# totokunda/apex-studio

Measured on AMD Instinct MI355X. Metric: denoise_steps_per_sec, higher is better.
Workload: dtype bf16; 1 GPU; flux-dev-1024x1024 denoise step (19 double + 38 single MM-DiT blocks, S_img 4096 + S_txt 512, B=1, no CFG) + FlowMatch-Euler step; clips_in_flight=1, parallelism=clip-per-gpu x1

## Files before the change

### apex-studio_amd/csrc/common.h

```cpp
#pragma once
#include <hip/hip_runtime.h>
#include <stdint.h>
#include <stddef.h>

#include "../../include/apexmi.h"

typedef __attribute__((ext_vector_type(8))) __bf16 bf16x8;
typedef __attribute__((ext_vector_type(4))) __bf16 bf16x4;
typedef __attribute__((ext_vector_type(2))) __bf16 bf16x2;
typedef __attribute__((ext_vector_type(16))) float f32x16;
typedef __attribute__((ext_vector_type(4))) float f32x4;
typedef __attribute__((ext_vector_type(2))) float f32x2;
typedef __attribute__((ext_vector_type(4))) uint32_t u32x4;
typedef __attribute__((ext_vector_type(2))) uint32_t u32x2;

typedef uint16_t bf16_t;

#define APEXMI_DEVICE __device__ __forceinline__

APEXMI_DEVICE float bf16_lo(uint32_t u) { return __uint_as_float(u << 16); }
APEXMI_DEVICE float bf16_hi(uint32_t u) { return __uint_as_float(u & 0xffff0000u); }
APEXMI_DEVICE float bf16_to_f32(bf16_t b) { return __uint_as_float((uint32_t)b << 16); }

APEXMI_DEVICE uint32_t pack_bf16(float a, float b) {
// ... 123 lines not shown
}
APEXMI_DEVICE float sum_xor32(float x) {
    float a, b;
    swap32(x, a, b);
    return a + b;
}

APEXMI_DEVICE float wave_sum(float x) {
#pragma unroll
    for (int o = 32; o > 0; o >>= 1) x += __shfl_xor(x, o, 64);
    return x;
}
APEXMI_DEVICE float wave_max(float x) {
#pragma unroll
    for (int o = 32; o > 0; o >>= 1) x = fmaxf(x, __shfl_xor(x, o, 64));
    return x;
}

APEXMI_DEVICE float fast_exp2(float x) { return __builtin_amdgcn_exp2f(x); }
APEXMI_DEVICE float x_sigmoid_log2(float x, float z_log2) {
    return x * __builtin_amdgcn_rcpf(1.0f + __builtin_amdgcn_exp2f(-z_log2));
}
APEXMI_DEVICE float silu_f(float x) { return x_sigmoid_log2(x, 1.4426950408889634f * x); }
APEXMI_DEVICE float gelu_tanh_f(float x) {
    const float a = 2.0f * 0.7978845608028654f * 1.4426950408889634f, b = a * 0.044715f;
    return x_sigmoid_log2(x, x * fmaf(b, x * x, a));
}

APEXMI_DEVICE void glds16(const void* gsrc, void* lds) {
    __builtin_amdgcn_global_load_lds((const __attribute__((address_space(1))) void*)gsrc,
                                     (__attribute__((address_space(3))) void*)lds, 16, 0, 0);
}

APEXMI_DEVICE int xcd_remap(int bid, int total) {
    const int q = total >> 3, r = total & 7;
    const int xcd = bid & 7, idx = bid >> 3;
    const int base = (xcd < r) ? xcd * (q + 1) : r * (q + 1) + (xcd - r) * q;
    return base + idx;
}

static inline bool apexmi_attr_needed(const uint64_t& mask) {
    int dev = 0;
    (void)hipGetDevice(&dev);
    return dev >= 64 || !(__atomic_load_n(&mask, __ATOMIC_ACQUIRE) & (1ull << dev));
}
static inline void apexmi_attr_done(uint64_t& mask) {
    int dev = 0;
    (void)hipGetDevice(&dev);
    if (dev < 64) (void)__atomic_fetch_or(&mask, 1ull << dev, __ATOMIC_RELEASE);
}
#define APEXMI_SET_ATTR_ONCE(mask, ...)      \
    do {                                     \
        if (apexmi_attr_needed(mask)) {      \
            __VA_ARGS__;                     \
            apexmi_attr_done(mask);          \
        }                                    \
    } while (0)
void apexmi_set_error(const char* fmt, ...);
int apexmi_check_launch(const char* what);
__attribute__((visibility("hidden"))) int apexmi_attn_merge_f32(int n, const float* parts, const float* lses, void* out,
                                                                 float* lse_out, int B, int H, int Sq, int D,
                                                                 const int64_t* o_strides, const int64_t* lse_strides, int dtype,
                                                                 hipStream_t stream);
unsigned long long* apexmi_clk_ptr();

struct ApexmiProfScope {
    int cls;
// ... 14 lines not shown
```

### apex-studio_amd/csrc/gemm.hip

```cpp
#include "common.h"

#include <cstring>
#include <type_traits>

namespace {

#ifndef APEXMI_GEMM_TRACE
#define APEXMI_GEMM_TRACE 0
#endif
#define PP_BAR()                               \
    do {                                       \
        __builtin_amdgcn_sched_barrier(0);     \
        __builtin_amdgcn_s_barrier();          \
        __builtin_amdgcn_sched_barrier(0);     \
    } while (0)
#define PP_SYNC()                                                                   \
    do {                                                                            \
        asm volatile("s_waitcnt lgkmcnt(0)" ::: "memory");                          \
        PP_BAR();                                                                   \
    } while (0)
#define VMCNT(n) asm volatile("s_waitcnt vmcnt(" #n ")" ::: "memory")
constexpr int BK = 64;
constexpr int GROUP_M = 6;
constexpr int EPI_GATE_RES_F32 = 7;
constexpr int MAX_GROUPS = 4;

struct GemmProblem {
    const bf16_t* A;
    const bf16_t* W;
    const bf16_t* bias;
    bf16_t* C;
    const float* gate;
    const bf16_t* R;
    int64_t lda, ldw, ldc, ldr;
    int M, N, nm, nn, tile0, gelu;
    int qkv, row0;
    const bf16_t* nq;
    const bf16_t* nk;
};
struct QkvShared {
    bf16_t* qo;
    bf16_t* ko;
    bf16_t* vt;
    const float* rope;
    int S_out, Skp, inner;
    float eps;
    const float* rope_pairs;
};
struct GemmGroup {
    GemmProblem p[MAX_GROUPS];
    int count, K, total, group_m;
    int batch;
    int64_t bsA, bsW, bsC_bytes;
    QkvShared qs;
    unsigned long long* clk;
#if APEXMI_GEMM_TRACE
    unsigned long long* trace;
#endif
    int wpacked;
};

template <int BM_, int BN_, int WM_, int WN_, int SCHED_>
struct Cfg {
    static constexpr int BM = BM_, BN = BN_, WM = WM_, WN = WN_;
    static constexpr int SCHED = SCHED_;
    static constexpr bool PP = SCHED_ == 1;
    static constexpr int NW = WM * WN, NT = NW * 64;
    static constexpr int TM = BM / WM / 32, TN = BN / WN / 32;
    static constexpr int A_BYTES = BM * BK * 2, W_BYTES = BN * BK * 2;
    static constexpr int STAGE = A_BYTES + W_BYTES;
    static constexpr int LDS = SCHED_ == 8 ? 5 * 32768 : 2 * STAGE;
    static constexpr int A_LD = BM * 8 / NT, W_LD = BN * 8 / NT;
    static constexpr int OCC = (LDS <= 80 * 1024 && NT == 256) ? 2 : (NT == 512 ? 2 : 1);
};
using CFG_128 = Cfg<128, 128, 2, 2, 0>;
using CFG_256 = Cfg<256, 256, 2, 4, 0>;
using CFG_128E = Cfg<128, 128, 2, 4, 0>;
using CFG_256P = Cfg<256, 256, 2, 4, 1>;
using CFG_256W = Cfg<256, 256, 2, 2, 4>;
using CFG_256P16 = Cfg<256, 256, 2, 4, 5>;
using CFG_256R = Cfg<256, 256, 2, 4, 7>;
using CFG_256R5 = Cfg<256, 256, 2, 4, 8>;

APEXMI_DEVICE float act_f(float x, int mode) {
    if (mode == 1) return gelu_tanh_f(x);
    if (mode == 2) return 0.5f * x * (1.0f + erff(x * 0.70710678118654752f));
    if (mode == 4) return x_sigmoid_log2(x, (1.702f * 1.4426950408889634f) * x);
    return silu_f(x);
}
template <int ACT>
APEXMI_DEVICE float act_c(float x) {
    if constexpr (ACT == 0) return x;
// ... 473 lines not shown
            if (!(APEXMI_QK_ABL & 16) && (MT > 8 || (mt & 1))) __builtin_amdgcn_sched_barrier(0);
        }
    }
}

#if APEXMI_GEMM_TRACE
#define APEXMI_TRACE_END()                                                                                   \
    do {                                                                                                     \
        if (G.trace != nullptr) {                                                                            \
            __builtin_amdgcn_sched_barrier(0);                                                               \
            const unsigned long long t_st = __builtin_amdgcn_s_memrealtime();                                \
            asm volatile("s_waitcnt vmcnt(0)" ::: "memory");                                                 \
            const unsigned long long t_ack = __builtin_amdgcn_s_memrealtime();                               \
            if (tid == 0) {                                                                                  \
                unsigned long long* o = G.trace + (size_t)blockIdx.x * 8;                                    \
                o[0] = __builtin_amdgcn_s_getreg((31 << 11) | (0 << 6) | 4);               \
                o[1] = __builtin_amdgcn_s_getreg((31 << 11) | (0 << 6) | 20);             \
                o[2] = tr_in;                                                                                \
                o[3] = tr_l0;                                                                                \
                o[4] = tr_l1;                                                                                \
                o[5] = t_st;                                                                                 \
                o[6] = t_ack;                                                                                \
                o[7] = (unsigned long long)s;                                                                \
            }                                                                                                \
        }                                                                                                    \
    } while (0)
#else
#define APEXMI_TRACE_END() do { } while (0)
#endif

struct TileCoord {
    int pm, pn;
};
__device__ __forceinline__ TileCoord tile_coord(int s, int nm, int nn, int group_m) {
    const int width = group_m * nn;
    const int first_m = (s / width) * group_m;
    const int gsz = min(nm - first_m, group_m);
    return TileCoord{first_m + (s % width) % gsz, (s % width) / gsz};
}

__device__ __forceinline__ const char* uniform_ptr(const char* p) {
    const uint64_t u = (uint64_t)p;
    const uint32_t hi = __builtin_amdgcn_readfirstlane((uint32_t)(u >> 32)), lo = __builtin_amdgcn_readfirstlane((uint32_t)u);
    return (const char*)(((uint64_t)hi << 32) | lo);
}
#pragma clang diagnostic push
#pragma clang diagnostic ignored "-Winline-asm"
__device__ __forceinline__ void glds16_s(const char* sbase, uint32_t voff, uint32_t la) {
    asm volatile("s_mov_b32 m0, %2\n\ts_nop 0\n\tglobal_load_lds_dwordx4 %0, %1"
                 :: "v"(voff), "s"(sbase), "s"(la) : "memory", "m0");
}
#pragma clang diagnostic pop

struct KRange {
    int kt0, kt1;
};
template <typename CFG, int EPI>
__device__ __forceinline__ void gemm_tile(const GemmGroup& G, char* smem, int s, const KRange& kr) {
    constexpr int BM = CFG::BM, BN = CFG::BN, TM = CFG::TM, TN = CFG::TN;

#if APEXMI_GEMM_TRACE
    unsigned long long tr_in = 0, tr_l0 = 0, tr_l1 = 0;
    if (G.trace != nullptr) tr_in = __builtin_amdgcn_s_memrealtime();
#endif
    int tid_ = threadIdx.x;
    asm volatile("" : "+v"(tid_));
    const int tid = tid_;
    const int lane = tid & 63;
    const int wave = __builtin_amdgcn_readfirstlane(tid >> 6);
    const int wm = wave / CFG::WN, wn = wave % CFG::WN;
    const int l31 = lane & 31, hi = lane >> 5;
// ... 814 lines not shown
    }
    const int nbase = n0 + wn * 48;
    if constexpr (EPI == APEXMI_EPI_BIAS_GATE_RES) {
        u32x4 rr[9];
        u32x2 r1[9];
        const int nst = nbase + 16 * (g4 & 1) + 8 * (g4 >> 1);
#pragma unroll
        for (int mt = 0; mt < 9; ++mt) {
            const bf16_t* row = P.R + (int64_t)max(mrow[mt], 0) * P.ldr;
            rr[mt] = *(const u32x4*)(row + min(nst, N - 8));
            r1[mt] = *(const u32x2*)(row + min(nbase + 32 + 4 * g4, N - 4));
        }
        store_slab16<EPI, 9, 0>(acc[0], acc[1], P, N, mrow, nbase, g4, rr);
        store_single16<EPI, 9, 0>(acc[2], P, N, mrow, nbase + 32, g4, r1);
    } else {
        APEXMI_ACT_DISPATCH(P.gelu, store_slab16<EPI, 9, ACT>(acc[0], acc[1], P, N, mrow, nbase, g4);
                            store_single16<EPI, 9, ACT>(acc[2], P, N, mrow, nbase + 32, g4, nullptr));
    }
}

constexpr int YBM = 384, YBN = 256;
constexpr int Y_A_BYTES = YBM * BK * 2, Y_W_BYTES = YBN * BK * 2, Y_STAGE = Y_A_BYTES + Y_W_BYTES, Y_LDS = 2 * Y_STAGE;

template <int EPI, int DIST = 1, int QKV = 0>
__global__ __launch_bounds__(512, 2) void gemm_bf16_x384_kernel(const GemmGroup G) {
    extern __shared__ __attribute__((aligned(16))) char smem[];
    const int tid = threadIdx.x;
    const int lane = tid & 63;
    const int wave = __builtin_amdgcn_readfirstlane(tid >> 6);
    const int wm = wave >> 2, wn = wave & 3;

    int s = xcd_remap(blockIdx.x, G.total);
    int gi = 0;
#pragma unroll
    for (int i = 1; i < MAX_GROUPS; ++i)
        if (i < G.count && s >= G.p[i].tile0) gi = i;
    const GemmProblem P = G.p[gi];
    s -= P.tile0;
    const int N = P.N, M = P.M;
    const TileCoord tc = tile_coord(s, P.nm, P.nn, G.group_m);
    const int m0 = tc.pm * YBM, n0 = tc.pn * YBN;

    const int rows_a = min(M - m0, YBM), rows_w = min(N - n0, YBN);
    auto rsrc_a = __builtin_amdgcn_make_buffer_rsrc((void*)(P.A + (int64_t)m0 * P.lda), 0,
                                                    (int)(((int64_t)(rows_a - 1) * P.lda + G.K) * 2), 0x00020000);
    auto rsrc_w = __builtin_amdgcn_make_buffer_rsrc((void*)(P.W + (int64_t)n0 * P.ldw), 0,
                                                    (int)(((int64_t)(rows_w - 1) * P.ldw + G.K) * 2), 0x00020000);
    const int par = wave & 1, widx = wave >> 1;
    const int sw_src = ((lane & 7) ^ (4 * par + (lane >> 4))) * 16;
    const int voff_a = (lane >> 3) * (int)P.lda * 2 + sw_src;
    const int voff_w = (lane >> 3) * (int)P.ldw * 2 + sw_src;
    const int lda8 = (int)P.lda * 16, ldw8 = (int)P.ldw * 16;
    auto piece_of = [&](int j) -> int {
        if (j < 4) return 2 * (4 * j + widx) + par;
        const int e = 3 * widx + (j < 7 ? j - 4 : j - 7);
        return (e < 6 ? 0 : 24) + (j < 7 ? 0 : 12) + 2 * (e % 6) + par;
    };
    auto stage = [&](int buf, int kt, int j) {
        const int pc = piece_of(j);
        char* dst = smem + buf * Y_STAGE + (j < 4 ? Y_A_BYTES : 0) + pc * 1024;
        if (j < 4)
            __builtin_amdgcn_raw_ptr_buffer_load_lds(rsrc_w, (__attribute__((address_space(3))) void*)dst, 16, voff_w, pc * ldw8 + kt * (BK * 2), 0, 0);
        else
            __builtin_amdgcn_raw_ptr_buffer_load_lds(rsrc_a, (__attribute__((address_space(3))) void*)dst, 16, voff_a, pc * lda8 + kt * (BK * 2), 0, 0);
    };

    f32x4_t acc[4][12];
#pragma unroll
    for (int i = 0; i < 4; ++i)
#pragma unroll
        for (int j = 0; j < 12; ++j) acc[i][j] = f32x4_t{0.f, 0.f, 0.f, 0.f};

    const int nkt = G.K / BK;
// ... 135 lines not shown
        }
#pragma unroll
        for (int p = 0; p < 2; ++p) {
            const int nbase = n0 + wn * 64 + p * 32;
            const f32x4_t(&x)[MTC] = *(const f32x4_t(*)[MTC]) & acc[2 * p][h * MTC];
            const f32x4_t(&y)[MTC] = *(const f32x4_t(*)[MTC]) & acc[2 * p + 1][h * MTC];
            if constexpr (EPI == APEXMI_EPI_BIAS_GATE_RES) {
                u32x4 rr[MTC];
                const int nst = nbase + 16 * (g4 & 1) + 8 * (g4 >> 1);
#pragma unroll
                for (int mt = 0; mt < MTC; ++mt) rr[mt] = *(const u32x4*)(P.R + (int64_t)max(mrow[mt], 0) * P.ldr + min(nst, N - 8));
                store_slab16<EPI, MTC, 0>(x, y, P, N, mrow, nbase, g4, rr);
            } else {
                APEXMI_ACT_DISPATCH(P.gelu, store_slab16<EPI, MTC, ACT>(x, y, P, N, mrow, nbase, g4));
            }
        }
    }
    Y_TRACE_END(3);
}
#undef Y_TRACE_END

int g_group_m = GROUP_M;
#if APEXMI_GEMM_TRACE
uintptr_t g_gemm_trace = 0;
#endif
int g_large_cfg = 7;
int g_force_cfg = 0;
int g_wpacked = 0;
int g_tail_max = 96;
int g_x288 = 0;
int g_x384_group_m = 3;
int g_x384_dist = -1;
int g_x384_qkv = 1;
int g_x384 = 1;
int g_small_max = 112;
int g_tail_split = 2;

int number_tiles(GemmGroup& G, const int* Ms, int BM, int BN) {
    int t = 0;
    for (int i = 0; i < G.count; ++i) {
        G.p[i].M = Ms[i];
        G.p[i].nm = (Ms[i] + BM - 1) / BM;
        G.p[i].nn = (G.p[i].N + BN - 1) / BN;
        G.p[i].tile0 = t;
        t += G.p[i].nm * G.p[i].nn;
    }
    G.total = t;
    G.clk = apexmi_clk_ptr();
#if APEXMI_GEMM_TRACE
    G.trace = (unsigned long long*)g_gemm_trace;
#endif
    G.wpacked = 0;
    return t;
}

template <typename CFG, int EPI>
int launch_cfg(GemmGroup& G, const int* Ms, hipStream_t stream) {
    if constexpr (CFG::SCHED == 0 || CFG::SCHED == 5) {
        for (int i = 0; i < G.count; ++i)
            if (G.p[i].lda > (1 << 22) || G.p[i].ldw > (1 << 22)) {
                apexmi_set_error("gemm_bf16: leading dimensions above 2^22 elements are not supported (lda %lld, ldw %lld)",
                                 (long long)G.p[i].lda, (long long)G.p[i].ldw);
                return 1;
            }
    }
    static uint64_t attr_set = 0;
    APEXMI_SET_ATTR_ONCE(attr_set,
        (void)hipFuncSetAttribute((const void*)gemm_bf16_kernel<CFG, EPI>,
                                  hipFuncAttributeMaxDynamicSharedMemorySize, CFG::LDS));
    const int t = number_tiles(G, Ms, CFG::BM, CFG::BN);
    G.group_m = g_group_m;
    if (CFG::SCHED == 5) G.wpacked = g_wpacked;
    hipLaunchKernelGGL((gemm_bf16_kernel<CFG, EPI>), dim3(t, G.batch), dim3(CFG::NT), CFG::LDS, stream, G);
    return apexmi_check_launch("gemm_bf16");
}

template <int EPI>
int launch_x288(GemmGroup& G, const int* Ms, hipStream_t stream) {
    static uint64_t attr_set = 0;
    APEXMI_SET_ATTR_ONCE(attr_set,
        (void)hipFuncSetAttribute((const void*)gemm_bf16_x288_kernel<EPI>, hipFuncAttributeMaxDynamicSharedMemorySize, X_LDS));
    const int t = number_tiles(G, Ms, XBM, XBN);
    G.group_m = g_group_m;
    hipLaunchKernelGGL((gemm_bf16_x288_kernel<EPI>), dim3(t, 1), dim3(512), X_LDS, stream, G);
    return apexmi_check_launch("gemm_bf16 (288x192)");
}

template <int EPI>
int launch_x384(GemmGroup& G, const int* Ms, hipStream_t stream) {
    static uint64_t attr_set = 0;
    APEXMI_SET_ATTR_ONCE(attr_set,
        (void)hipFuncSetAttribute((const void*)gemm_bf16_x384_kernel<EPI, 0>, hipFuncAttributeMaxDynamicSharedMemorySize, Y_LDS);
        (void)hipFuncSetAttribute((const void*)gemm_bf16_x384_kernel<EPI, 1>, hipFuncAttributeMaxDynamicSharedMemorySize, Y_LDS);
        if constexpr (EPI == APEXMI_EPI_BIAS)
            (void)hipFuncSetAttribute((const void*)gemm_bf16_x384_kernel<EPI, 1, 1>, hipFuncAttributeMaxDynamicSharedMemorySize, Y_LDS));
    const int t = number_tiles(G, Ms, YBM, YBN);
    G.group_m = g_x384_group_m;
    bool any_qkv = false;
    for (int i = 0; i < G.count; ++i) any_qkv |= G.p[i].qkv != 0;
    if constexpr (EPI == APEXMI_EPI_BIAS) {
        if (any_qkv) {
            hipLaunchKernelGGL((gemm_bf16_x384_kernel<EPI, 1, 1>), dim3(t, 1), dim3(512), Y_LDS, stream, G);
            return apexmi_check_launch("gemm_bf16 (384x256, fused q/k/v)");
        }
    }
    const int dist = g_x384_dist >= 0 ? g_x384_dist : (t >= 2048 ? 0 : 1);
    if (dist == 0) hipLaunchKernelGGL((gemm_bf16_x384_kernel<EPI, 0>), dim3(t, 1), dim3(512), Y_LDS, stream, G);
    else hipLaunchKernelGGL((gemm_bf16_x384_kernel<EPI, 1>), dim3(t, 1), dim3(512), Y_LDS, stream, G);
    return apexmi_check_launch("gemm_bf16 (384x256)");
}

inline bool x288_pays(const GemmGroup& G, const int* Ms) {
    int64_t t256 = 0, t288 = 0;
    for (int i = 0; i < G.count; ++i) {
        if (G.p[i].qkv) return false;
        t256 += (int64_t)((Ms[i] + 255) / 256) * ((G.p[i].N + 255) / 256);
        t288 += (int64_t)((Ms[i] + XBM - 1) / XBM) * ((G.p[i].N + XBN - 1) / XBN);
    }
    const double c256 = (double)((t256 + 255) / 256) * 65536.0;
    const double c288 = (double)((t288 + 255) / 256) * (XBM * XBN) * 1.04;
    return c288 < 0.95 * c256;
}

inline bool use_x288(const GemmGroup& G, const int* Ms) {
    if (g_x288 == 0 || G.batch != 1 || G.K % BK != 0 || !(g_force_cfg == 0 || g_force_cfg == 7) || g_large_cfg != 7) return false;
    int64_t mtot = 0;
    int nmax = 0;
    for (int i = 0; i < G.count; ++i) {
        if (G.p[i].qkv) return false;
        mtot += Ms[i];
        nmax = G.p[i].N > nmax ? G.p[i].N : nmax;
    }
    if (g_x288 == 2) return true;
    return G.K >= 256 && mtot >= 1024 && nmax >= 1024 && x288_pays(G, Ms);
// ... 178 lines not shown
    double flops = 0, bytes = 0;
    const int kind = epi_kind(epilogue[0]);
    for (int i = 0; i < count; ++i) {
        APEXMI_REQUIRE(epi_kind(epilogue[i]) == kind,
                       "gemm_bf16_grouped: gate/residual (or float / bf16 output) problems cannot be mixed with the others");
        const float* g = gate ? gate[i] : nullptr;
        const void* r = R ? R[i] : nullptr;
        const int64_t lr = ldr ? ldr[i] : 0;
        if (int rc = check_problem(A[i], lda[i], W[i], ldw[i], C[i], ldc[i], M[i], N[i], K, epilogue[i], g, r, lr))
            return rc;
        G.p[i] = GemmProblem{(const bf16_t*)A[i], (const bf16_t*)W[i], (const bf16_t*)(bias ? bias[i] : nullptr),
                             (bf16_t*)C[i], g, (const bf16_t*)r, lda[i], ldw[i], ldc[i], lr, M[i], N[i], 0, 0, 0,
                             act_mode(epi_base(epilogue[i]))};
        flops += 2.0 * M[i] * N[i] * (double)K;
        bytes += 2.0 * ((double)M[i] * K + (double)N[i] * K + (double)M[i] * N[i]);
    }
    ApexmiProfScope prof(0, stream, flops, bytes);
    return launch_group(G, M, kind, stream);
}

extern "C" int apexmi_gemm_uses_x288(int M, int N, int K) {
    GemmGroup G;
    memset(&G, 0, sizeof(G));
    G.count = 1;
    G.K = K;
    G.batch = 1;
    G.p[0].N = N;
    return (M > 0 && N > 0 && K > 0 && use_x288(G, &M)) ? 1 : 0;
}

extern "C" int apexmi_gemm_qkv_fusable(int64_t m_total, int n_max, int K) {
    return (g_force_cfg == 0 || g_force_cfg == 7 || g_force_cfg == 9 || g_force_cfg == 10) &&
           (g_large_cfg == 7 || g_large_cfg == 9 || g_large_cfg == 10) && m_total >= 1024 && n_max >= 1024 && K >= 256 && K % BK == 0;
}

extern "C" int apexmi_gemm_bf16_grouped_qkv(int count, const void* const* A, const int64_t* lda, const void* const* W,
                                            const int64_t* ldw, const void* const* bias, void* const* C, const int64_t* ldc,
                                            const int* M, const int* N, int K, const int* epilogue, const int* is_qkv,
                                            const void* const* norm_q, const void* const* norm_k, const int* row0, int H,
                                            float eps, const float* rope, void* q_out, void* k_out, void* vt_out, int S_out,
                                            int Skp, apexmi_stream_t stream_) {
    return apexmi_gemm_bf16_grouped_qkv_pairs(count, A, lda, W, ldw, bias, C, ldc, M, N, K, epilogue, is_qkv, norm_q, norm_k, row0, H,
                                              eps, rope, nullptr, q_out, k_out, vt_out, S_out, Skp, stream_);
}

extern "C" int apexmi_gemm_bf16_grouped_qkv_pairs(int count, const void* const* A, const int64_t* lda, const void* const* W,
                                                  const int64_t* ldw, const void* const* bias, void* const* C, const int64_t* ldc,
                                                  const int* M, const int* N, int K, const int* epilogue, const int* is_qkv,
                                                  const void* const* norm_q, const void* const* norm_k, const int* row0, int H,
                                                  float eps, const float* rope, const float* rope_pairs, void* q_out, void* k_out,
                                                  void* vt_out, int S_out, int Skp, apexmi_stream_t stream_) {
    hipStream_t stream = (hipStream_t)stream_;
    APEXMI_REQUIRE(((uintptr_t)rope_pairs % 16) == 0, "gemm_bf16_grouped_qkv: rope_pairs must be 16-byte aligned");
    APEXMI_REQUIRE(count >= 1 && count <= MAX_GROUPS, "gemm_bf16_grouped_qkv: count=%d not in [1,%d]", count, MAX_GROUPS);
    APEXMI_REQUIRE(is_qkv && row0 && rope && q_out && k_out && vt_out && H > 0, "gemm_bf16_grouped_qkv: null argument");
    APEXMI_REQUIRE(H % 2 == 0 && S_out > 0 && Skp >= S_out && Skp % 8 == 0, "gemm_bf16_grouped_qkv: H=%d must be even, Skp=%d a multiple of 8 >= S_out=%d",
                   H, Skp, S_out);
    APEXMI_REQUIRE(((uintptr_t)rope % 16) == 0 && ((uintptr_t)q_out % 16) == 0 && ((uintptr_t)k_out % 16) == 0 && ((uintptr_t)vt_out % 16) == 0,
                   "gemm_bf16_grouped_qkv: rope / outputs must be 16-byte aligned");
    GemmGroup G;
    G.count = count;
    G.K = K;
    G.batch = 1;
    G.bsA = G.bsW = G.bsC_bytes = 0;
    G.qs = QkvShared{(bf16_t*)q_out, (bf16_t*)k_out, (bf16_t*)vt_out, rope, S_out, Skp, H * 128, eps, rope_pairs};
    double flops = 0, bytes = 0;
// ... 33 lines not shown
        return launch_x384<APEXMI_EPI_BIAS>(G, M, stream);
    if (g_large_cfg == 9 || g_force_cfg == 9) return launch_cfg<CFG_256R, APEXMI_EPI_BIAS>(G, M, stream);
    if (g_large_cfg == 10 || g_force_cfg == 10) return launch_cfg<CFG_256R5, APEXMI_EPI_BIAS>(G, M, stream);
    return launch_cfg<CFG_256P16, APEXMI_EPI_BIAS>(G, M, stream);
}

extern "C" int apexmi_split_bf16x3(const float* x, int64_t ldx, int64_t M, int K, void* out, int64_t ldo,
                                   apexmi_stream_t stream_) {
    hipStream_t stream = (hipStream_t)stream_;
    APEXMI_REQUIRE(x && out && M > 0 && K > 0, "split_bf16x3: bad arguments");
    APEXMI_REQUIRE(K % 8 == 0 && ldx % 4 == 0 && ldo % 8 == 0 && ldo >= 3 * (int64_t)K && ((uintptr_t)x % 16) == 0 &&
                       ((uintptr_t)out % 16) == 0,
                   "split_bf16x3: K=%d must be a multiple of 8 and rows 16-byte aligned", K);
    const int64_t n = M * (K / 8);
    ApexmiProfScope prof(5, stream, 0.0, 10.0 * (double)M * K);
    hipLaunchKernelGGL(split_bf16x3_kernel, dim3((unsigned)((n + 255) / 256)), dim3(256), 0, stream, x, ldx, M, K,
                       (bf16_t*)out, ldo);
    return apexmi_check_launch("split_bf16x3");
}

int apexmi_set_gemm_key(const char* key, int value) {
    if (!strcmp(key, "gemm.tail")) g_tail_split = value;
    else if (!strcmp(key, "gemm.tail_max")) g_tail_max = value;
    else if (!strcmp(key, "gemm.group_m")) g_group_m = value > 0 ? value : GROUP_M;
    else if (!strcmp(key, "gemm.large")) g_large_cfg = value;
    else if (!strcmp(key, "gemm.config")) g_force_cfg = value;
    else if (!strcmp(key, "gemm.wpacked")) g_wpacked = value;
    else if (!strcmp(key, "gemm.x288")) g_x288 = value;
    else if (!strcmp(key, "gemm.small_max")) g_small_max = value;
    else if (!strcmp(key, "gemm.x384")) g_x384 = value;
    else if (!strcmp(key, "gemm.x384_dist")) g_x384_dist = value;
    else if (!strcmp(key, "gemm.x384_group_m")) g_x384_group_m = value > 0 ? value : 3;
    else if (!strcmp(key, "gemm.x384_qkv")) g_x384_qkv = value;
#if APEXMI_GEMM_TRACE
    else if (!strcmp(key, "gemm.trace_lo")) g_gemm_trace = (g_gemm_trace & ~(uintptr_t)0xffffffffu) | (uint32_t)value;
    else if (!strcmp(key, "gemm.trace_hi")) g_gemm_trace = (g_gemm_trace & (uintptr_t)0xffffffffu) | ((uintptr_t)(uint32_t)value << 32);
#endif
    else return 1;
    return 0;
}
```

### apex-studio_amd/lib.py

```python
from __future__ import annotations

import ctypes as C
import os

_PKG_DIR = os.path.dirname(os.path.abspath(__file__))
LIB_PATH = os.environ.get("APEX_MI355_LIB") or os.path.join(_PKG_DIR, "libapex_mi355.so")

_lib = None

c_i64p = C.POINTER(C.c_int64)
c_f32p = C.c_void_p
vp = C.c_void_p

SIGNATURES = {
    "apexmi_version": (C.c_int, []),
    "apexmi_last_error": (C.c_char_p, []),
    "apexmi_attn_workspace_bytes": (C.c_size_t, [C.c_int] * 6),
    "apexmi_attn_fwd": (C.c_int, [vp, vp, vp, vp, C.c_int, C.c_int, C.c_int, C.c_int, C.c_int,
                                  c_i64p, c_i64p, c_i64p, c_i64p, C.c_float, C.c_int, vp,
                                  C.c_size_t, vp]),
    "apexmi_attn_fwd_prepared": (C.c_int, [vp, vp, vp, vp, C.c_int, C.c_int, C.c_int, C.c_int,
                                           C.c_int, c_i64p, C.c_float, vp]),
    "apexmi_attn_prepared_workspace_bytes": (C.c_size_t, [C.c_int] * 4),
    "apexmi_attn_fwd_prepared_ws": (C.c_int, [vp, vp, vp, vp, C.c_int, C.c_int, C.c_int, C.c_int,
# ... 15 lines not shown
                                                                                                C.c_float, C.c_int, vp, C.c_size_t, vp]),
    "apexmi_attn_merge": (C.c_int, [C.c_int, C.POINTER(vp), C.POINTER(vp), vp, vp] + [C.c_int] * 4 + [c_i64p, c_i64p, C.c_int, vp]),
    "apexmi_attn_varlen_workspace_bytes": (C.c_size_t, [C.c_int] * 4),
    "apexmi_attn_fwd_varlen": (C.c_int, [vp] * 7 + [C.c_int] * 8 + [c_i64p] * 5 + [C.c_int, C.c_float, C.c_int, vp, C.c_size_t, vp]),
    "apexmi_attn_window_map_bytes": (C.c_size_t, [C.c_int, C.c_int]),
    "apexmi_attn_window_map": (C.c_int, [vp, vp] + [C.c_int] * 5 + [vp, C.c_size_t, vp]),
    "apexmi_attn_fwd_window": (C.c_int, [vp, vp, vp, vp] + [C.c_int] * 6 + [c_i64p] * 4 + [vp, vp, C.c_int, C.c_int, C.c_int, vp,
                                                                                        C.c_float, C.c_int, vp, C.c_size_t, vp]),
    "apexmi_attn_fwd_prepared_window": (C.c_int, [vp, vp, vp, vp] + [C.c_int] * 5 + [c_i64p, vp, vp, C.c_int, C.c_int, C.c_int, vp,
                                                                                     C.c_float, vp]),
    "apexmi_attn_fwd_prepared_band": (C.c_int, [vp, vp, vp, vp] + [C.c_int] * 5 + [c_i64p, vp, C.c_int, C.c_float, vp]),
    "apexmi_attn_band_workspace_bytes": (C.c_size_t, [C.c_int] * 4),
    "apexmi_attn_fwd_band": (C.c_int, [vp, vp, vp, vp] + [C.c_int] * 5 + [c_i64p] * 4 + [vp, C.c_int, C.c_float, C.c_int, vp,
                                                                                      C.c_size_t, vp]),
    "apexmi_attn_fwd_prepared_dual": (C.c_int, [vp, vp, vp, C.c_int, C.c_int, vp, vp, C.c_int, C.c_int, vp, C.c_int, C.c_int,
                                                C.c_int, c_i64p, C.c_float, vp]),
    "apexmi_gemm_bf16": (C.c_int, [vp, C.c_int64, vp, C.c_int64, vp, vp, C.c_int64, C.c_int, C.c_int,
                                   C.c_int, C.c_int, vp, vp, C.c_int64, vp]),
    "apexmi_gemm_bf16_grouped": (C.c_int, [C.c_int, C.POINTER(vp), c_i64p, C.POINTER(vp), c_i64p,
                                           C.POINTER(vp), C.POINTER(vp), c_i64p, C.POINTER(C.c_int),
                                           C.POINTER(C.c_int), C.c_int, C.POINTER(C.c_int), C.POINTER(vp),
                                           C.POINTER(vp), c_i64p, vp]),
    "apexmi_gemm_bf16_grouped_qkv": (C.c_int, [C.c_int, C.POINTER(vp), c_i64p, C.POINTER(vp), c_i64p, C.POINTER(vp),
                                               C.POINTER(vp), c_i64p, C.POINTER(C.c_int), C.POINTER(C.c_int), C.c_int,
                                               C.POINTER(C.c_int), C.POINTER(C.c_int), C.POINTER(vp), C.POINTER(vp),
                                               C.POINTER(C.c_int), C.c_int, C.c_float, vp, vp, vp, vp, C.c_int, C.c_int, vp]),
    "apexmi_gemm_bf16_grouped_qkv_pairs": (C.c_int, [C.c_int, C.POINTER(vp), c_i64p, C.POINTER(vp), c_i64p, C.POINTER(vp),
                                                     C.POINTER(vp), c_i64p, C.POINTER(C.c_int), C.POINTER(C.c_int), C.c_int,
                                                     C.POINTER(C.c_int), C.POINTER(C.c_int), C.POINTER(vp), C.POINTER(vp),
                                                     C.POINTER(C.c_int), C.c_int, C.c_float, vp, vp, vp, vp, vp, C.c_int, C.c_int, vp]),
    "apexmi_rope_pairs": (C.c_int, [vp, C.c_int, C.c_int, vp, vp, vp]),
    "apexmi_gemm_qkv_fusable": (C.c_int, [C.c_int64, C.c_int, C.c_int]),
    "apexmi_gemm_uses_x288": (C.c_int, [C.c_int, C.c_int, C.c_int]),
    "apexmi_qk_rms_rope_rows": (C.c_int, [vp, vp, vp, C.c_int64, C.c_int, C.c_int, vp, vp, C.c_float, vp, C.c_int, vp, vp, vp,
                                          C.c_int, C.c_int, C.c_int, vp]),
    "apexmi_qk_rms_rope_rows_f32": (C.c_int, [vp, vp, vp, C.c_int64, C.c_int, C.c_int, vp, vp, C.c_float, vp, C.c_int, vp, vp, vp,
                                              C.c_int, C.c_int, C.c_int, vp]),
    "apexmi_gemm_bf16_batched": (C.c_int, [vp, C.c_int64, C.c_int64, vp, C.c_int64, C.c_int64, vp, C.c_int64, C.c_int64,
                                           C.c_int, C.c_int, C.c_int, C.c_int, C.c_int, vp]),
    "apexmi_attn_bias_workspace_bytes": (C.c_size_t, [C.c_int] * 4),
    "apexmi_attn_fwd_bias": (C.c_int, [vp, C.c_int64, vp, C.c_int64, vp, C.c_int64, vp, C.c_int64, C.c_int, C.c_int,
                                       C.c_int, C.c_int, C.c_int, C.c_float, vp, vp, vp, C.c_int, vp, C.c_size_t, vp]),
    "apexmi_rope_half": (C.c_int, [vp, C.c_int64, C.c_int64, C.c_int, C.c_int, C.c_int, vp, vp, vp]),
    "apexmi_rope_half_f32": (C.c_int, [vp, C.c_int64, C.c_int64, C.c_int, C.c_int, C.c_int, vp, vp, vp]),
    "apexmi_tune_set": (C.c_int, [C.c_char_p, C.c_int]),
    "apexmi_gemv": (C.c_int, [vp, C.c_int64, vp, vp, C.c_int64, vp, C.c_int64, C.c_int, C.c_int,
                              C.c_int, C.c_int, vp]),
    "apexmi_ln_modulate": (C.c_int, [vp, C.c_int64, vp, C.c_int64, C.c_int, C.c_int, vp, vp, vp, vp,
                                     C.c_float, C.c_int, vp]),
    "apexmi_ln_modulate2": (C.c_int, [vp, C.c_int64, vp, C.c_int64, C.c_int, C.c_int, vp, vp, vp, vp,
                                      C.c_float, C.c_int, C.c_int, vp, vp, vp]),
    "apexmi_qkv_prepare": (C.c_int, [vp, vp, vp, C.c_int64, C.c_int, C.c_int, C.c_int, C.c_int, vp, vp,
                                     vp, vp, C.c_float, vp, C.c_int, vp, vp, vp, C.c_int, C.c_int,
                                     C.c_int, vp]),
    "apexmi_v_transpose": (C.c_int, [vp, C.c_int64, C.c_int64, C.c_int, C.c_int, C.c_int, vp, C.c_int,
                                     C.c_int, vp]),
    "apexmi_conv3d_cl": (C.c_int, [vp, vp, vp, vp, vp, vp] + [C.c_int] * 9 + [vp]),
    "apexmi_conv3d_cl_replicate": (C.c_int, [vp, vp, vp, vp, vp, vp] + [C.c_int] * 9 + [vp]),
    "apexmi_conv3d_cl_clips": (C.c_int, [vp, vp, vp, vp, vp, vp] + [C.c_int] * 11 + [vp]),
    "apexmi_conv3d_cl_strided": (C.c_int, [vp, vp, vp, vp, vp, vp] + [C.c_int] * 15 + [vp]),
    "apexmi_conv3d_cl_frames": (C.c_int, [vp, vp, vp, vp, vp, vp] + [C.c_int] * 9 + [vp]),
    "apexmi_conv3d_cl_up2": (C.c_int, [vp, vp, vp, vp, vp, vp] + [C.c_int] * 10 + [vp]),
    "apexmi_conv3d_cl_norm_fusable": (C.c_int, [C.c_int] * 6),
    "apexmi_conv3d_cl_family": (C.c_int, [C.c_int] * 23 + [vp]),
    "apexmi_conv3d_cl_norm": (C.c_int, [vp, vp, vp, vp, vp, vp, vp, C.c_int, vp] + [C.c_int] * 11 + [vp]),
    "apexmi_add_bf16": (C.c_int, [vp, vp, vp, C.c_int64, vp]),
# ... 155 lines not shown
```

### include/apexmi.h

```cpp
#ifndef APEXMI_H
#define APEXMI_H

#include <stdint.h>
#include <stddef.h>

#ifdef __cplusplus
extern "C" {
#endif

typedef void* apexmi_stream_t;

#define APEXMI_BF16 0
#define APEXMI_F16 1
#define APEXMI_F32 2
#define APEXMI_MASK_BOOL 3

#define APEXMI_EPI_BIAS 0
#define APEXMI_EPI_BIAS_GELU 1
#define APEXMI_EPI_BIAS_GATE_RES 2
#define APEXMI_EPI_BIAS_GELU_ERF 4
#define APEXMI_EPI_BIAS_QUICK_GELU 6
#define APEXMI_EPI_BIAS_SILU 5
#define APEXMI_EPI_BIAS_F32 3

// ... 83 lines not shown
                           const int64_t o_strides[3], const void* q_coords, const void* k_coords, int r0, int r1, int r2,
                           const void* map, float softmax_scale, int dtype, void* workspace, size_t workspace_bytes,
                           apexmi_stream_t stream);
int apexmi_attn_fwd_prepared_window(const void* q, const void* k, const void* vt, void* out, int B, int H, int Sq, int Sk,
                                    int Skp, const int64_t o_strides[3], const void* q_coords, const void* k_coords, int r0,
                                    int r1, int r2, const void* map, float softmax_scale, apexmi_stream_t stream);

int apexmi_attn_fwd_prepared_band(const void* q, const void* k, const void* vt, void* out, int B, int H, int Sq, int Sk,
                                  int Skp, const int64_t o_strides[3], const void* bands, int Hb, float softmax_scale,
                                  apexmi_stream_t stream);
size_t apexmi_attn_band_workspace_bytes(int B, int H, int Sq, int Sk);
int apexmi_attn_fwd_band(const void* q, const void* k, const void* v, void* out, int B, int H, int Sq, int Sk, int D,
                         const int64_t q_strides[3], const int64_t k_strides[3], const int64_t v_strides[3],
                         const int64_t o_strides[3], const void* bands, int Hb, float softmax_scale, int dtype,
                         void* workspace, size_t workspace_bytes, apexmi_stream_t stream);

int apexmi_attn_fwd_prepared_dual(const void* q, const void* k_t, const void* vt_t, int Sk_t, int Skp_t, const void* k_i,
                                  const void* vt_i, int Sk_i, int Skp_i, void* out, int B, int H, int Sq,
                                  const int64_t o_strides[3], float softmax_scale, apexmi_stream_t stream);

int apexmi_gemm_bf16(const void* A, int64_t lda, const void* W, int64_t ldw, const void* bias,
                     void* C, int64_t ldc, int M, int N, int K, int epilogue,
                     const float* gate, const void* R, int64_t ldr, apexmi_stream_t stream);

int apexmi_gemm_uses_x288(int M, int N, int K);

int apexmi_gemm_bf16_grouped(int count, const void* const* A, const int64_t* lda,
                             const void* const* W, const int64_t* ldw, const void* const* bias,
                             void* const* C, const int64_t* ldc, const int* M, const int* N, int K,
                             const int* epilogue, const float* const* gate, const void* const* R,
                             const int64_t* ldr, apexmi_stream_t stream);

int apexmi_gemm_qkv_fusable(int64_t m_total, int n_max, int K);
int apexmi_gemm_bf16_grouped_qkv(int count, const void* const* A, const int64_t* lda, const void* const* W,
                                 const int64_t* ldw, const void* const* bias, void* const* C, const int64_t* ldc,
                                 const int* M, const int* N, int K, const int* epilogue, const int* is_qkv,
                                 const void* const* norm_q, const void* const* norm_k, const int* row0, int H, float eps,
                                 const float* rope, void* q_out, void* k_out, void* vt_out, int S_out, int Skp,
                                 apexmi_stream_t stream);
int apexmi_gemm_bf16_grouped_qkv_pairs(int count, const void* const* A, const int64_t* lda, const void* const* W,
                                       const int64_t* ldw, const void* const* bias, void* const* C, const int64_t* ldc,
                                       const int* M, const int* N, int K, const int* epilogue, const int* is_qkv,
                                       const void* const* norm_q, const void* const* norm_k, const int* row0, int H, float eps,
                                       const float* rope, const float* rope_pairs, void* q_out, void* k_out, void* vt_out,
                                       int S_out, int Skp, apexmi_stream_t stream);
int apexmi_rope_pairs(const float* rope, int S, int D, float* pairs, int* mismatch, apexmi_stream_t stream);

int apexmi_split_bf16x3(const float* x, int64_t ldx, int64_t M, int K, void* out, int64_t ldo, apexmi_stream_t stream);

int apexmi_gemm_bf16_batched(const void* A, int64_t lda, int64_t stride_a, const void* W, int64_t ldw, int64_t stride_w,
                             void* C, int64_t ldc, int64_t stride_c, int batch, int M, int N, int K, int epilogue,
                             apexmi_stream_t stream);

size_t apexmi_attn_bias_workspace_bytes(int H, int Sq, int Sk, int D);
int apexmi_attn_fwd_bias(const void* q, int64_t ldq, const void* k, int64_t ldk, const void* v, int64_t ldv, void* out,
                         int64_t ldo, int H, int Hkv, int Sq, int Sk, int D, float softmax_scale, const float* bias,
                         const uint8_t* keep, const int* seg, int causal, void* workspace, size_t workspace_bytes,
                         apexmi_stream_t stream);

int apexmi_tune_set(const char* key, int value);

int apexmi_gemv(const void* W, int64_t ldw, const void* bias, const float* x, int64_t ldx,
                float* y, int64_t ldy, int M, int N, int K, int flags, apexmi_stream_t stream);

int apexmi_ln_modulate(const void* x, int64_t ldx, void* out, int64_t ldo, int M, int C,
                       const float* scale, const float* shift, const void* gamma,
// ... 191 lines not shown
```

Measured before the change: 16.69 steps/s.

## Schedule Q/K tiles before V tiles in fused grouped QKV GEMM

Renumbers the tiles of the fused QKV grouped GEMM so that all Q and K column tiles, across groups, are dispatched first and the V/remaining tiles afterwards, each set with its own XCD remap. The aim is to have the Q/K tiles, which feed the fused RMS-norm/RoPE epilogue, finish earlier and balance the heavier epilogue tiles across the grid, which may reduce tail imbalance. A host-callable mapping function is added for testing. It adds a little index arithmetic per block and may change L2 reuse patterns.

```diff
diff --git a/apex-studio_amd/csrc/common.h b/apex-studio_amd/csrc/common.h
--- a/apex-studio_amd/csrc/common.h
+++ b/apex-studio_amd/csrc/common.h
@@ -179,7 +179,7 @@
                                      (__attribute__((address_space(3))) void*)lds, 16, 0, 0);
 }
 
-APEXMI_DEVICE int xcd_remap(int bid, int total) {
+__host__ APEXMI_DEVICE int xcd_remap(int bid, int total) {
     const int q = total >> 3, r = total & 7;
     const int xcd = bid & 7, idx = bid >> 3;
     const int base = (xcd < r) ? xcd * (q + 1) : r * (q + 1) + (xcd - r) * q;
diff --git a/apex-studio_amd/csrc/gemm.hip b/apex-studio_amd/csrc/gemm.hip
--- a/apex-studio_amd/csrc/gemm.hip
+++ b/apex-studio_amd/csrc/gemm.hip
@@ -1,5 +1,6 @@
 #include "common.h"
 
+#include <climits>
 #include <cstring>
 #include <type_traits>
 
@@ -58,6 +59,8 @@
     unsigned long long* trace;
 #endif
     int wpacked;
+    int n_first, nn_qk;
+    int first0[MAX_GROUPS];
 };
 
 template <int BM_, int BN_, int WM_, int WN_, int SCHED_>
@@ -597,11 +600,28 @@
 struct TileCoord {
     int pm, pn;
 };
-__device__ __forceinline__ TileCoord tile_coord(int s, int nm, int nn, int group_m) {
+__host__ __device__ __forceinline__ TileCoord tile_coord(int s, int nm, int nn, int group_m) {
     const int width = group_m * nn;
     const int first_m = (s / width) * group_m;
     const int gsz = min(nm - first_m, group_m);
     return TileCoord{first_m + (s % width) % gsz, (s % width) / gsz};
+}
+
+struct TileRef {
+    int gi, pm, pn;
+};
+__host__ __device__ __forceinline__ TileRef split_tile_ref(const GemmGroup& G, int bid) {
+    const bool first = bid < G.n_first;
+    int s = first ? xcd_remap(bid, G.n_first) : xcd_remap(bid - G.n_first, G.total - G.n_first);
+    int gi = 0;
+#pragma unroll
+    for (int i = 1; i < MAX_GROUPS; ++i)
+        if (i < G.count && s >= (first ? G.first0[i] : G.p[i].tile0)) gi = i;
+    s -= first ? G.first0[gi] : G.p[gi].tile0;
+    const bool cut = G.n_first > 0 && G.p[gi].qkv != 0;
+    const int nn = first ? G.nn_qk : cut ? G.p[gi].nn - G.nn_qk : G.p[gi].nn;
+    const TileCoord tc = tile_coord(s, G.p[gi].nm, nn, G.group_m);
+    return TileRef{gi, tc.pm, tc.pn + (!first && cut ? G.nn_qk : 0)};
 }
 
 __device__ __forceinline__ const char* uniform_ptr(const char* p) {
@@ -1482,13 +1502,22 @@
 
     int s = xcd_remap(blockIdx.x, G.total);
     int gi = 0;
-#pragma unroll
-    for (int i = 1; i < MAX_GROUPS; ++i)
-        if (i < G.count && s >= G.p[i].tile0) gi = i;
+    TileCoord tc;
+    if constexpr (QKV == 1) {
+        const TileRef tr = split_tile_ref(G, blockIdx.x);
+        gi = tr.gi;
+        tc = TileCoord{tr.pm, tr.pn};
+    } else {
+#pragma unroll
+        for (int i = 1; i < MAX_GROUPS; ++i)
+            if (i < G.count && s >= G.p[i].tile0) gi = i;
+    }
     const GemmProblem P = G.p[gi];
-    s -= P.tile0;
+    if constexpr (QKV != 1) {
+        s -= P.tile0;
+        tc = tile_coord(s, P.nm, P.nn, G.group_m);
+    }
     const int N = P.N, M = P.M;
-    const TileCoord tc = tile_coord(s, P.nm, P.nn, G.group_m);
     const int m0 = tc.pm * YBM, n0 = tc.pn * YBN;
 
     const int rows_a = min(M - m0, YBM), rows_w = min(N - n0, YBN);
@@ -1690,6 +1719,7 @@
 int g_x384_group_m = 3;
 int g_x384_dist = -1;
 int g_x384_qkv = 1;
+int g_qk_first = 1;
 int g_x384 = 1;
 int g_small_max = 112;
 int g_tail_split = 2;
@@ -1709,7 +1739,23 @@
     G.trace = (unsigned long long*)g_gemm_trace;
 #endif
     G.wpacked = 0;
+    G.n_first = G.nn_qk = 0;
+    for (int i = 0; i < MAX_GROUPS; ++i) G.first0[i] = INT_MAX;
     return t;
+}
+
+void number_tiles_qk_first(GemmGroup& G, int nn_qk) {
+    int ta = 0, tb = 0;
+    for (int i = 0; i < G.count; ++i) {
+        GemmProblem& p = G.p[i];
+        const int qk = p.qkv ? nn_qk : 0;
+        G.first0[i] = qk ? ta : INT_MAX;
+        p.tile0 = tb;
+        ta += p.nm * qk;
+        tb += p.nm * (p.nn - qk);
+    }
+    G.n_first = ta;
+    G.nn_qk = nn_qk;
 }
 
 template <typename CFG, int EPI>
@@ -1758,6 +1804,7 @@
     for (int i = 0; i < G.count; ++i) any_qkv |= G.p[i].qkv != 0;
     if constexpr (EPI == APEXMI_EPI_BIAS) {
         if (any_qkv) {
+            if (g_qk_first) number_tiles_qk_first(G, 2 * G.qs.inner / YBN);
             hipLaunchKernelGGL((gemm_bf16_x384_kernel<EPI, 1, 1>), dim3(t, 1), dim3(512), Y_LDS, stream, G);
             return apexmi_check_launch("gemm_bf16 (384x256, fused q/k/v)");
         }
@@ -2002,6 +2049,34 @@
 extern "C" int apexmi_gemm_qkv_fusable(int64_t m_total, int n_max, int K) {
     return (g_force_cfg == 0 || g_force_cfg == 7 || g_force_cfg == 9 || g_force_cfg == 10) &&
            (g_large_cfg == 7 || g_large_cfg == 9 || g_large_cfg == 10) && m_total >= 1024 && n_max >= 1024 && K >= 256 && K % BK == 0;
+}
+
+extern "C" int apexmi_gemm_qk_first_map(int count, const int* nm, const int* nn, const int* is_qkv, int nn_qk, int group_m,
+                                        int qk_first, int* out) {
+    if (count < 1 || count > MAX_GROUPS || !nm || !nn || !is_qkv || !out || group_m < 1 || nn_qk < 1) return -1;
+    GemmGroup G;
+    memset(&G, 0, sizeof(G));
+    G.count = count;
+    G.group_m = group_m;
+    int t = 0;
+    for (int i = 0; i < count; ++i) {
+        if (nm[i] < 1 || nn[i] < 1 || (is_qkv[i] && nn_qk >= nn[i])) return -1;
+        G.p[i].nm = nm[i];
+        G.p[i].nn = nn[i];
+        G.p[i].qkv = is_qkv[i] ? 1 : 0;
+        G.p[i].tile0 = t;
+        G.first0[i] = INT_MAX;
+        t += nm[i] * nn[i];
+    }
+    G.total = t;
+    if (qk_first) number_tiles_qk_first(G, nn_qk);
+    for (int b = 0; b < t; ++b) {
+        const TileRef r = split_tile_ref(G, b);
+        out[3 * b] = r.gi;
+        out[3 * b + 1] = r.pm;
+        out[3 * b + 2] = r.pn;
+    }
+    return G.n_first;
 }
 
 extern "C" int apexmi_gemm_bf16_grouped_qkv(int count, const void* const* A, const int64_t* lda, const void* const* W,
@@ -2101,6 +2176,7 @@
     else if (!strcmp(key, "gemm.x384_dist")) g_x384_dist = value;
     else if (!strcmp(key, "gemm.x384_group_m")) g_x384_group_m = value > 0 ? value : 3;
     else if (!strcmp(key, "gemm.x384_qkv")) g_x384_qkv = value;
+    else if (!strcmp(key, "gemm.qk_first")) g_qk_first = value;
 #if APEXMI_GEMM_TRACE
     else if (!strcmp(key, "gemm.trace_lo")) g_gemm_trace = (g_gemm_trace & ~(uintptr_t)0xffffffffu) | (uint32_t)value;
     else if (!strcmp(key, "gemm.trace_hi")) g_gemm_trace = (g_gemm_trace & (uintptr_t)0xffffffffu) | ((uintptr_t)(uint32_t)value << 32);
diff --git a/apex-studio_amd/lib.py b/apex-studio_amd/lib.py
--- a/apex-studio_amd/lib.py
+++ b/apex-studio_amd/lib.py
@@ -71,6 +71,8 @@
     "apexmi_rope_pairs": (C.c_int, [vp, C.c_int, C.c_int, vp, vp, vp]),
     "apexmi_gemm_qkv_fusable": (C.c_int, [C.c_int64, C.c_int, C.c_int]),
     "apexmi_gemm_uses_x288": (C.c_int, [C.c_int, C.c_int, C.c_int]),
+    "apexmi_gemm_qk_first_map": (C.c_int, [C.c_int, C.POINTER(C.c_int), C.POINTER(C.c_int), C.POINTER(C.c_int), C.c_int, C.c_int,
+                                           C.c_int, C.POINTER(C.c_int)]),
     "apexmi_qk_rms_rope_rows": (C.c_int, [vp, vp, vp, C.c_int64, C.c_int, C.c_int, vp, vp, C.c_float, vp, C.c_int, vp, vp, vp,
                                           C.c_int, C.c_int, C.c_int, vp]),
     "apexmi_qk_rms_rope_rows_f32": (C.c_int, [vp, vp, vp, C.c_int64, C.c_int, C.c_int, vp, vp, C.c_float, vp, C.c_int, vp, vp, vp,
diff --git a/include/apexmi.h b/include/apexmi.h
--- a/include/apexmi.h
+++ b/include/apexmi.h
@@ -139,6 +139,8 @@
                              const int64_t* ldr, apexmi_stream_t stream);
 
 int apexmi_gemm_qkv_fusable(int64_t m_total, int n_max, int K);
+int apexmi_gemm_qk_first_map(int count, const int* nm, const int* nn, const int* is_qkv, int nn_qk, int group_m, int qk_first,
+                             int* out);
 int apexmi_gemm_bf16_grouped_qkv(int count, const void* const* A, const int64_t* lda, const void* const* W,
                                  const int64_t* ldw, const void* const* bias, void* const* C, const int64_t* ldc,
                                  const int* M, const int* N, int K, const int* epilogue, const int* is_qkv,
```

Result: no change. 16.73 steps/s (median of 4 runs) (+0.2%).
